# labhamlet/wavjepa

Measured on NVIDIA B200. Metric: WavJEPA-base train 2s-instances/s at 1/2/4/8 B200; tensor-pipe % of peak, higher is better.
Workload: dtype bf16

## Files before the change

include/wavjepa_b200.h:

```cpp
#ifndef WAVJEPA_B200_H
#define WAVJEPA_B200_H

#include <stddef.h>
#include <stdint.h>

#ifdef __cplusplus
extern "C" {
#endif

#define WJ_OK 0
#define WJ_ERR_ARG (-1)
#define WJ_ERR_RUNTIME (-2)
#define WJ_ERR_ARCH (-3)

const char* wj_last_error(void);
int wj_version(void);
long long wj_kernel_launches(void);
int wj_check_device(void);

typedef struct wj_operand {
  const void* ptr;
  int64_t dim[4];
  int64_t stride_bytes[3];
  int32_t seg_width;
// ... 13 lines not shown
  int32_t resid_f32;
  int32_t resid_mod;
  int64_t ld_resid;
  const void* aux;
  int64_t ld_aux;
  int32_t act;
  int32_t _pad;
  const int32_t* out_rows;
  float* colsum;
} wj_epilogue_t;

int wj_gemm_bf16(const wj_operand_t* A, const void* W, int64_t ldw, int L, int batch, int N, int K,
                 const wj_epilogue_t* epi, int block_n, void* stream);

int wj_gemm_dgrad_bf16(const wj_operand_t* A, const void* W, int64_t ldw, int w_rows, int w_cols,
                       const int32_t* seg_col_off, int L, int batch, int N, int K, const wj_epilogue_t* epi,
                       int block_n, void* stream);

int wj_set_deterministic(void* workspace, size_t bytes);

int wj_gemm_option(int key, int value);

int wj_gemm_debug(void* counters);

int wj_gemm_wgrad_bf16(const wj_operand_t* dY, const wj_operand_t* X, int L, int batch, int M, int N, float* out,
                       int64_t ld_out, int accumulate, int splits, void* stream);

int wj_masks_generate(int kind, int batch, int n_times, int in_channels, int channel_based, int n_targets,
                      double ctx_prob, int ctx_len, double tgt_prob, int tgt_len, float cutoff, int min_context_len,
                      uint32_t base_seed, uint32_t row0, uint8_t* ctx_hidden, uint8_t* tgt, uint8_t* vis_hidden,
                      int* attempts, int* err_flag, void* stream);

int wj_mask_indices(const uint8_t* ctx_hidden, const uint8_t* tgt, const uint8_t* vis_hidden, int B, int G, int T,
                    int* n_c, int* n_v, int* n_t, int* cu_c, int* cu_v, int* cu_t, int* totals, int* ctx_rows,
                    int* vis_src, int* vis_pos, int* tgt_vrow, int* tgt_trow, void* stream);

int wj_conv0_moment_count(int Cin);
int wj_conv0_gn_gelu_fwd(const void* x_bf16, const float* w, const float* gamma, const float* beta, int B, int Cin,
                         int L, int C, int k, int stride, float eps, double* moments, float* stats, void* out_bf16,
                         void* dgelu_bf16, void* stream);
int wj_conv0_gn_gelu_bwd(const void* x_bf16, const float* w, const float* gamma, const float* beta, int B, int Cin,
                         int L, int C, int k, int stride, float eps, const double* moments, const float* stats,
                         const void* dy_bf16, const void* dgelu_bf16, void* red_scratch, float* dw, float* dgamma,
                         float* dbeta, void* stream);

int wj_layernorm_fwd(const void* x, int x_is_bf16, const float* gamma, const float* beta, float eps, int M, int D,
// ... 91 lines not shown
```

wavjepa_b200/csrc/attention.cu:

```cuda
#include "common.cuh"

namespace wj {

__device__ __forceinline__ void mma16816(float (&c)[4], const uint32_t (&a)[4], uint32_t b0, uint32_t b1) {
  asm volatile(
      "mma.sync.aligned.m16n8k16.row.col.f32.bf16.bf16.f32 {%0,%1,%2,%3}, {%4,%5,%6,%7}, {%8,%9}, {%0,%1,%2,%3};"
      : "+f"(c[0]), "+f"(c[1]), "+f"(c[2]), "+f"(c[3])
      : "r"(a[0]), "r"(a[1]), "r"(a[2]), "r"(a[3]), "r"(b0), "r"(b1));
}
__device__ __forceinline__ void ldsm_x4_trans(uint32_t& r0, uint32_t& r1, uint32_t& r2, uint32_t& r3, const void* p) {
  asm volatile("ldmatrix.sync.aligned.m8n8.x4.trans.shared.b16 {%0,%1,%2,%3}, [%4];"
               : "=r"(r0), "=r"(r1), "=r"(r2), "=r"(r3)
               : "r"(smem_u32(p)));
}
__device__ __forceinline__ uint32_t lds32(const bf16* p) { return *reinterpret_cast<const uint32_t*>(p); }

__device__ __forceinline__ void ldsm_x4(uint32_t& r0, uint32_t& r1, uint32_t& r2, uint32_t& r3, const void* p) {
  asm volatile("ldmatrix.sync.aligned.m8n8.x4.shared.b16 {%0,%1,%2,%3}, [%4];"
               : "=r"(r0), "=r"(r1), "=r"(r2), "=r"(r3)
               : "r"(smem_u32(p)));
}
__device__ __forceinline__ void cp_async16(void* dst, const void* src) {
  asm volatile("cp.async.cg.shared.global [%0], [%1], 16;" ::"r"(smem_u32(dst)), "l"(src) : "memory");
}
// ... 369 lines not shown

extern "C" int wj_attn_varlen_bwd(const void* qkv_bf16, const void* out_bf16, const void* dout_bf16, const float* lse2,
                                  const int* cu_seqlens, int n_seqs, int max_len, int64_t total_tokens, int D, int H,
                                  void* dqkv_bf16, void* stream) {
  return wj_attn_varlen_bwd_bias(qkv_bf16, out_bf16, dout_bf16, lse2, cu_seqlens, n_seqs, max_len, total_tokens, D, H,
                                 dqkv_bf16, nullptr, stream);
}

static int attn_bwd_bias(const void* qkv_bf16, const void* out_bf16, const void* dout_bf16, const float* lse2,
                         const int* cu_seqlens, int n_seqs, int max_len, int64_t total_tokens, int D, int H,
                         void* dqkv_bf16, float* dbias, void* stream, bool allow_rowstats) {
  if (n_seqs <= 0 || max_len <= 0) return WJ_OK;
  const int dh = D / H;
  if (D % H != 0 || (dh != 32 && dh != 64)) { set_error("wj_attn_varlen_bwd: head dim must be 32 or 64"); return WJ_ERR_ARG; }
  {
    const bool det = wj::det_on();
    const int rc = wj::attn_bwd_tc_launch(qkv_bf16, out_bf16, dout_bf16, lse2, cu_seqlens, n_seqs, max_len, total_tokens, D, H,
                                          dqkv_bf16, det ? nullptr : dbias, WJ_STREAM(stream));
    if (rc < 0) return rc;
    if (rc == 0 && det) {
      if (dbias != nullptr) return wj_colsum(dqkv_bf16, 1, total_tokens, 3 * D, 3 * D, dbias, stream);
      return WJ_OK;
    }
    if (rc == 0) {
      if (dbias != nullptr) return wj_colsum(dout_bf16, 1, total_tokens, D, D, dbias + 2 * D, stream);
      return WJ_OK;
    }
  }
  const int npad = (max_len + 15) & ~15;
  size_t smem = static_cast<size_t>(4) * npad * (dh + 8) * 2 + static_cast<size_t>(2) * ((npad + 63) & ~63) * 4;
  const bool rowstats = allow_rowstats && dh == 64 && smem > 227 * 1024;
  if (rowstats) smem = static_cast<size_t>(4) * npad * (dh + 8) * 2;
  if (smem > 227 * 1024) { set_error("wj_attn_varlen_bwd: sequence of %d tokens (head dim %d) exceeds the shared-memory resident design", max_len, dh); return WJ_ERR_ARG; }
  const float scale = 1.0f / sqrtf(static_cast<float>(dh));
  const float scale_log2 = scale * 1.4426950408889634f;
  dim3 grid(H, n_seqs);
  const bf16* q = reinterpret_cast<const bf16*>(qkv_bf16);
  const bf16* o = reinterpret_cast<const bf16*>(out_bf16);
  const bf16* d_o = reinterpret_cast<const bf16*>(dout_bf16);
  bf16* dq = reinterpret_cast<bf16*>(dqkv_bf16);
  cudaError_t e;
  if (rowstats) {
    e = cudaFuncSetAttribute(attn_bwd_kernel<64, true>, cudaFuncAttributeMaxDynamicSharedMemorySize, static_cast<int>(smem));
    if (e != cudaSuccess) { set_error("attn_bwd attr: %s", cudaGetErrorString(e)); return WJ_ERR_RUNTIME; }
    attn_bwd_kernel<64, true><<<grid, 128, smem, WJ_STREAM(stream)>>>(q, o, d_o, lse2, cu_seqlens, D, H, npad, scale, scale_log2, dq);
  } else if (dh == 64) {
    e = cudaFuncSetAttribute(attn_bwd_kernel<64>, cudaFuncAttributeMaxDynamicSharedMemorySize, static_cast<int>(smem));
    if (e != cudaSuccess) { set_error("attn_bwd attr: %s", cudaGetErrorString(e)); return WJ_ERR_RUNTIME; }
    attn_bwd_kernel<64><<<grid, 128, smem, WJ_STREAM(stream)>>>(q, o, d_o, lse2, cu_seqlens, D, H, npad, scale, scale_log2, dq);
  } else {
// ... 24 lines not shown
```

wavjepa_b200/csrc/attention_tc.cu:

```cuda
#include "common.cuh"

namespace wj {

constexpr int kAtQ = 128;
constexpr int kAtK = 128;

struct AttnTcParams {
  const int* cu;
  int n_seqs, D, H, items;
  float scale_log2;
  bf16* out;
  float* lse2;
  float* out_f32;
};

template <int DH, int KT> struct AttnTcCfg {
  static constexpr int TILE = kAtQ * DH * 2;
  static constexpr int HALVES = KT / 128;
  static constexpr int NW = 4 * HALVES;
  static constexpr int THREADS = (NW + 1) * 32;
  static constexpr int STAGE = 3 * HALVES * TILE;
  static constexpr int STAGES = DH == 32 ? 2 : 1;
  static constexpr int BAR_OFF = STAGES * STAGE;
  static constexpr int ML_OFF = BAR_OFF + 128;
// ... 316 lines not shown
          w.y = pack_bf16x2(__uint_as_float(o[j + 2]) * inv, __uint_as_float(o[j + 3]) * inv);
          w.z = pack_bf16x2(__uint_as_float(o[j + 4]) * inv, __uint_as_float(o[j + 5]) * inv);
          w.w = pack_bf16x2(__uint_as_float(o[j + 6]) * inv, __uint_as_float(o[j + 7]) * inv);
          *reinterpret_cast<uint4*>(op + j) = w;
        }
        if (p.lse2 != nullptr && half == 0) p.lse2[static_cast<long long>(start + row) * p.H + head] = mtot + log2f(lsum);
      }
      }
    }
  }
  tc_fence_before();
  __syncthreads();
  if (warp == NW) {
    tc_fence_after();
    tmem_dealloc(tmem_base, KT);
  }
}

struct AttnBwdParams {
  const int* cu;
  int D, H, items;
  float scale, scale_log2;
  const bf16* out;
  const bf16* dout;
  const float* lse2;
  bf16* dqkv;
  float* dbias;
};

constexpr int kBwdTile = kAtQ * 32 * 2;
constexpr int kBwdPs = 2 * kAtQ * 128;
constexpr int kBwdBarOff = 5 * kBwdTile + 2 * kBwdPs;
constexpr int kBwdCsOff = kBwdBarOff + 128;
constexpr int kBwdCsMaxD = 1024;
constexpr int kBwdSmem = kBwdCsOff + kBwdCsMaxD * 4 + 1024;

__global__ void __launch_bounds__(288, 2) attn_bwd_tc_kernel(const __grid_constant__ CUtensorMap tmQ,
                                                             const __grid_constant__ CUtensorMap tmDO,
                                                             const __grid_constant__ CUtensorMap tmO, const AttnBwdParams p) {
  constexpr int DH = 32;
  constexpr uint32_t SWZ = 4u, SBO = 512u;
  extern __shared__ uint8_t smem_raw[];
  uint8_t* smem = reinterpret_cast<uint8_t*>((reinterpret_cast<uintptr_t>(smem_raw) + 1023) & ~uintptr_t(1023));
  uint8_t* sP = smem + 5 * kBwdTile;
  uint8_t* sDS = sP + kBwdPs;
  uint64_t* bar_load = reinterpret_cast<uint64_t*>(smem + kBwdBarOff);
  uint64_t* bar_s = bar_load + 1;
  uint64_t* bar_p = bar_load + 2;
  uint64_t* bar_g = bar_load + 3;
  uint64_t* bar_done = bar_load + 4;
  uint32_t* tmem_slot = reinterpret_cast<uint32_t*>(bar_load + 5);
  float* s_cs = reinterpret_cast<float*>(smem + kBwdCsOff);
  const int warp = threadIdx.x >> 5, lane = threadIdx.x & 31;
  if (p.dbias != nullptr)
    for (int i = threadIdx.x; i < p.D; i += blockDim.x) s_cs[i] = 0.f;

  if (warp == 8) {
    if (lane == 0) {
      tma_prefetch_desc(&tmQ);
      tma_prefetch_desc(&tmDO);
      tma_prefetch_desc(&tmO);
      mbar_init(bar_load, 1);
      mbar_init(bar_s, 1);
      mbar_init(bar_p, 8);
      mbar_init(bar_g, 1);
      mbar_init(bar_done, 8);
      fence_mbar_init();
    }
    __syncwarp();
    tmem_alloc(tmem_slot, 256);
  }
  tc_fence_before();
  __syncthreads();
  tc_fence_after();
  const uint32_t tmem_base = *tmem_slot;
  const uint32_t tS = tmem_base, tDP = tmem_base + 128, tDV = tmem_base, tDK = tmem_base + 32, tDQ = tmem_base + 64;

  if (warp == 8) {
    if (lane == 0) {
      constexpr uint32_t idesc_g = umma_idesc_bf16(kAtQ, DH, true, true);
      constexpr uint32_t idesc_q = umma_idesc_bf16(kAtQ, DH, false, true);
      const uint32_t sQ = smem_u32(smem), sK = sQ + kBwdTile, sV = sK + kBwdTile, sDO = sV + kBwdTile;
      uint32_t ph_load = 0, ph_p = 0, ph_g = 0, ph_done = 0;
      int it = 0;
      for (int item = blockIdx.x; item < p.items; item += gridDim.x, ++it) {
        const int s = item / p.H, head = item - s * p.H;
        const int start = p.cu[s], n = p.cu[s + 1] - start;
        const int n16 = n > 0 ? (n + 15) & ~15 : 16;
        const uint32_t idesc_s = umma_idesc_bf16(kAtQ, n16, false, false);
        if (it > 0) {
          mbar_wait(bar_g, ph_g);
          ph_g ^= 1;
        }
        mbar_arrive_expect_tx(bar_load, 5 * kBwdTile);
        tma_load_2d(smem, &tmQ, bar_load, head * DH, start);
        tma_load_2d(smem + kBwdTile, &tmQ, bar_load, p.D + head * DH, start);
        tma_load_2d(smem + 2 * kBwdTile, &tmQ, bar_load, 2 * p.D + head * DH, start);
        tma_load_2d(smem + 3 * kBwdTile, &tmDO, bar_load, head * DH, start);
        tma_load_2d(smem + 4 * kBwdTile, &tmO, bar_load, head * DH, start);
        mbar_wait(bar_load, ph_load);
        ph_load ^= 1;
        if (it > 0) {
          mbar_wait(bar_done, ph_done);
          ph_done ^= 1;
        }
        tc_fence_after();
#pragma unroll
        for (int ks = 0; ks < DH / 16; ++ks)
          umma_bf16(tS, umma_smem_desc(sQ + ks * 32, 0, SBO, SWZ), umma_smem_desc(sK + ks * 32, 0, SBO, SWZ), idesc_s, ks > 0 ? 1u : 0u);
#pragma unroll
        for (int ks = 0; ks < DH / 16; ++ks)
          umma_bf16(tDP, umma_smem_desc(sDO + ks * 32, 0, SBO, SWZ), umma_smem_desc(sV + ks * 32, 0, SBO, SWZ), idesc_s, ks > 0 ? 1u : 0u);
        umma_commit(bar_s);
        if (item + gridDim.x < p.items) {
          const int nitem = item + gridDim.x, ns = nitem / p.H, nh = nitem - ns * p.H, nst = p.cu[ns];
          tma_prefetch_2d(&tmQ, nh * DH, nst);
          tma_prefetch_2d(&tmQ, p.D + nh * DH, nst);
          tma_prefetch_2d(&tmQ, 2 * p.D + nh * DH, nst);
          tma_prefetch_2d(&tmDO, nh * DH, nst);
          tma_prefetch_2d(&tmO, nh * DH, nst);
        }
        mbar_wait(bar_p, ph_p);
        ph_p ^= 1;
        tc_fence_after();
        const int steps = n16 / 16;
        const uint64_t dP_mn = umma_smem_desc(smem_u32(sP), kAtQ * 128, 1024, 2u);
        const uint64_t dS_mn = umma_smem_desc(smem_u32(sDS), kAtQ * 128, 1024, 2u);
        const uint64_t bDO = umma_smem_desc(sDO, kBwdTile, SBO, SWZ), bQ = umma_smem_desc(sQ, kBwdTile, SBO, SWZ),
                       bK = umma_smem_desc(sK, kBwdTile, SBO, SWZ);
        for (int kk = 0; kk < steps; ++kk)
          umma_bf16(tDV, dP_mn + static_cast<uint64_t>((kk * 2048) >> 4), bDO + static_cast<uint64_t>((kk * 1024) >> 4), idesc_g, kk > 0 ? 1u : 0u);
        for (int kk = 0; kk < steps; ++kk)
          umma_bf16(tDK, dS_mn + static_cast<uint64_t>((kk * 2048) >> 4), bQ + static_cast<uint64_t>((kk * 1024) >> 4), idesc_g, kk > 0 ? 1u : 0u);
        for (int kk = 0; kk < steps; ++kk) {
          const uint32_t a = smem_u32(sDS) + (kk >> 2) * (kAtQ * 128) + (kk & 3) * 32;
          umma_bf16(tDQ, umma_smem_desc(a, 0, 1024, 2u), bK + static_cast<uint64_t>((kk * 1024) >> 4), idesc_q, kk > 0 ? 1u : 0u);
        }
        umma_commit(bar_g);
      }
    }
  } else {
    const int quad = warp & 3, half = warp >> 2;
    const int row = quad * 32 + lane;
    const uint32_t lane_addr = static_cast<uint32_t>(quad * 32) << 16;
    uint8_t* stage = sP + half * (kAtQ * 128) + quad * 32 * 128;
    uint32_t ph_s = 0, ph_g = 0, ph_l = 0;
    int nstart = 0, nn = 0, n2start = 0, n2n = 0;
    float nlse = 0.f;
    if (blockIdx.x < p.items) {
      const int s = blockIdx.x / p.H;
      nstart = p.cu[s];
      nn = p.cu[s + 1] - nstart;
      if (row < nn) nlse = p.lse2[static_cast<long long>(nstart + row) * p.H + blockIdx.x % p.H];
    }
    if (blockIdx.x + gridDim.x < p.items) {
      const int s = (blockIdx.x + gridDim.x) / p.H;
      n2start = p.cu[s];
      n2n = p.cu[s + 1] - n2start;
    }
    const uint8_t* sOrow = smem + 4 * kBwdTile + row * 64;
    const uint8_t* sDOrow = smem + 3 * kBwdTile + row * 64;
    for (int item = blockIdx.x; item < p.items; item += gridDim.x) {
      const int head = item % p.H;
      const int start = nstart, n = nn;
      const float lse = nlse;
      nstart = n2start;
      nn = n2n;
      if (item + gridDim.x < p.items)
        nlse = row < nn ? p.lse2[static_cast<long long>(nstart + row) * p.H + (item + gridDim.x) % p.H] : 0.f;
      if (item + 2 * gridDim.x < p.items) {
        const int s = (item + 2 * gridDim.x) / p.H;
        n2start = p.cu[s];
        n2n = p.cu[s + 1] - n2start;
      }
      const bool live = row < n;
      mbar_wait(bar_load, ph_l);
      ph_l ^= 1;
      float delta = 0.f;
#pragma unroll
      for (int c = 0; c < 4; ++c) {
        const int o = (c ^ ((row >> 1) & 3)) << 4;
        const uint4 a = *reinterpret_cast<const uint4*>(sOrow + o);
        const uint4 b = *reinterpret_cast<const uint4*>(sDOrow + o);
        const __nv_bfloat162* a2 = reinterpret_cast<const __nv_bfloat162*>(&a);
        const __nv_bfloat162* b2 = reinterpret_cast<const __nv_bfloat162*>(&b);
#pragma unroll
        for (int t = 0; t < 4; ++t) {
          const float2 x = __bfloat1622float2(a2[t]), y = __bfloat1622float2(b2[t]);
          delta += x.x * y.x + x.y * y.y;
        }
      }
      mbar_wait(bar_s, ph_s);
      ph_s ^= 1;
      tc_fence_after();
#pragma unroll 1
      for (int c0 = half * 64; c0 < half * 64 + 64 && c0 < n; c0 += 32) {
        uint32_t sv[32], dv[32];
        tmem_ld_32x32(tS + lane_addr + c0, sv);
        tmem_ld_32x32(tDP + lane_addr + c0, dv);
        tmem_ld_wait();
        const int off = (c0 >> 6) * (kAtQ * 128) + row * 128;
#pragma unroll
        for (int q = 0; q < 4; ++q) {
          uint32_t wp[4], wd[4];
#pragma unroll
          for (int t = 0; t < 4; ++t) {
            const int j = q * 8 + 2 * t;
            const bool k0 = live && c0 + j < n, k1 = live && c0 + j + 1 < n;
            const float p0 = k0 ? ex2_approx(fmaf(__uint_as_float(sv[j]), p.scale_log2, -lse)) : 0.f;
            const float p1 = k1 ? ex2_approx(fmaf(__uint_as_float(sv[j + 1]), p.scale_log2, -lse)) : 0.f;
            wp[t] = pack_bf16x2(p0, p1);
            wd[t] = pack_bf16x2(k0 ? p0 * (__uint_as_float(dv[j]) - delta) : 0.f, k1 ? p1 * (__uint_as_float(dv[j + 1]) - delta) : 0.f);
          }
          const int chunk = ((c0 & 63) >> 3) + q;
          const int o = off + ((chunk ^ (row & 7)) << 4);
          *reinterpret_cast<uint4*>(sP + o) = make_uint4(wp[0], wp[1], wp[2], wp[3]);
          *reinterpret_cast<uint4*>(sDS + o) = make_uint4(wd[0], wd[1], wd[2], wd[3]);
        }
      }
      tc_fence_before();
      fence_proxy_async_smem();
      __syncwarp();
      if (lane == 0) mbar_arrive(bar_p);
      mbar_wait(bar_g, ph_g);
      ph_g ^= 1;
      tc_fence_after();
      const int ntile = half == 0 ? 2 : 1;
#pragma unroll
      for (int t = 0; t < 2; ++t) {
        if (t < ntile) {
          uint32_t g[32];
          tmem_ld_32x32((half == 0 ? (t == 0 ? tDQ : tDV) : tDK) + lane_addr, g);
          tmem_ld_wait();
          const float sc = (half == 0 && t == 1) ? 1.0f : p.scale;
#pragma unroll
          for (int q = 0; q < 4; ++q) {
            uint4 w;
            w.x = pack_bf16x2(__uint_as_float(g[8 * q]) * sc, __uint_as_float(g[8 * q + 1]) * sc);
            w.y = pack_bf16x2(__uint_as_float(g[8 * q + 2]) * sc, __uint_as_float(g[8 * q + 3]) * sc);
            w.z = pack_bf16x2(__uint_as_float(g[8 * q + 4]) * sc, __uint_as_float(g[8 * q + 5]) * sc);
            w.w = pack_bf16x2(__uint_as_float(g[8 * q + 6]) * sc, __uint_as_float(g[8 * q + 7]) * sc);
            *reinterpret_cast<uint4*>(stage + t * 2048 + lane * 64 + ((q ^ ((lane >> 1) & 3)) << 4)) = w;
          }
        }
      }
      if (p.dbias != nullptr && half == 1) {
        uint32_t g[32];
        tmem_ld_32x32(tDQ + lane_addr, g);
        tmem_ld_wait();
        float c32[32];
#pragma unroll
        for (int j = 0; j < 32; j += 2) {
          const uint32_t w = pack_bf16x2(__uint_as_float(g[j]) * p.scale, __uint_as_float(g[j + 1]) * p.scale);
          c32[j] = live ? __uint_as_float(w << 16) : 0.f;
          c32[j + 1] = live ? __uint_as_float(w & 0xffff0000u) : 0.f;
        }
#pragma unroll
        for (int sft = 16; sft >= 1; sft >>= 1) {
          const bool up = (lane & sft) != 0;
#pragma unroll
          for (int i = 0; i < sft; ++i) {
            const float mine = up ? c32[sft + i] : c32[i];
            const float other = up ? c32[i] : c32[sft + i];
            c32[i] = mine + __shfl_xor_sync(0xffffffffu, other, sft);
          }
        }
        atomicAdd(s_cs + head * DH + lane, c32[0]);
      }
      tc_fence_before();
      __syncwarp();
      if (lane == 0) mbar_arrive(bar_done);
      {
        const int rsub = lane >> 2, piece = lane & 3;
#pragma unroll
        for (int t = 0; t < 2; ++t) {
          if (t < ntile) {
            const int col = half == 0 ? (t == 0 ? 0 : 2 * p.D) : p.D;
#pragma unroll
            for (int r0 = 0; r0 < 32; r0 += 8) {
              const int lr = r0 + rsub, r = quad * 32 + lr;
              if (r < n) {
                const uint4 w = *reinterpret_cast<const uint4*>(stage + t * 2048 + lr * 64 + ((piece ^ ((lr >> 1) & 3)) << 4));
                *reinterpret_cast<uint4*>(p.dqkv + static_cast<long long>(start + r) * (3LL * p.D) + col + head * DH + piece * 8) = w;
              }
            }
          }
        }
      }
      __syncwarp();
    }
  }
  tc_fence_before();
  __syncthreads();
  if (p.dbias != nullptr)
    for (int i = threadIdx.x; i < p.D; i += blockDim.x) atomicAdd(p.dbias + i, s_cs[i]);
  if (warp == 8) {
    tc_fence_after();
    tmem_dealloc(tmem_base, 256);
  }
}

typedef CUresult (*PFN_encodeTiledA)(CUtensorMap*, CUtensorMapDataType, cuuint32_t, void*, const cuuint64_t*,
                                     const cuuint64_t*, const cuuint32_t*, const cuuint32_t*, CUtensorMapInterleave,
                                     CUtensorMapSwizzle, CUtensorMapL2promotion, CUtensorMapFloatOOBfill);

int attn_fwd_tc_launch(const void* qkv, const int* cu, int n_seqs, int max_len, long long total_tokens, int D, int H,
                       void* out, float* lse2, cudaStream_t st, float* out_f32) {
  const int dh = D / H;
  if (max_len > 512 || D % 64 != 0 || (dh != 32 && dh != 64) || total_tokens <= 0) return 1;
  static PFN_encodeTiledA enc = nullptr;
  if (enc == nullptr) {
    void* sym = nullptr;
    cudaDriverEntryPointQueryResult qres;
    if (cudaGetDriverEntryPoint("cuTensorMapEncodeTiled", &sym, cudaEnableDefault, &qres) != cudaSuccess ||
        qres != cudaDriverEntryPointSuccess)
      return 1;
    enc = reinterpret_cast<PFN_encodeTiledA>(sym);
  }
// ... 12 lines not shown
  p.out = reinterpret_cast<bf16*>(out); p.lse2 = lse2; p.out_f32 = out_f32;
  auto go = [&](auto kernel, int smem, int ctas, int threads) -> int {
    cudaError_t e = cudaFuncSetAttribute(kernel, cudaFuncAttributeMaxDynamicSharedMemorySize, smem);
    if (e != cudaSuccess) { set_error("attn_fwd_tc attr: %s", cudaGetErrorString(e)); return WJ_ERR_RUNTIME; }
    int grid = ctas * sm_count();
    if (grid > p.items) grid = p.items;
    kernel<<<grid, threads, smem, st>>>(tm, p);
    return check_launch("attn_fwd_tc");
  };
  if (out_f32 != nullptr) {
    if (dh != 64) { set_error("attn_fwd_tc: the fp32-output kernels are built for head dim 64 (got %d)", dh); return WJ_ERR_ARG; }
    if (qt == 4) return go(attn_fwd_tc_kernel<64, 512, true>, AttnTcCfg<64, 512>::SMEM, AttnTcCfg<64, 512>::CTAS, AttnTcCfg<64, 512>::THREADS);
    if (qt == 2) return go(attn_fwd_tc_kernel<64, 256, true>, AttnTcCfg<64, 256>::SMEM, AttnTcCfg<64, 256>::CTAS, AttnTcCfg<64, 256>::THREADS);
    return go(attn_fwd_tc_kernel<64, 128, true>, AttnTcCfg<64, 128>::SMEM, AttnTcCfg<64, 128>::CTAS, AttnTcCfg<64, 128>::THREADS);
  }
  if (dh == 64 && qt == 4) return go(attn_fwd_tc_kernel<64, 512>, AttnTcCfg<64, 512>::SMEM, AttnTcCfg<64, 512>::CTAS, AttnTcCfg<64, 512>::THREADS);
  if (qt == 4) return go(attn_fwd_tc_kernel<32, 512>, AttnTcCfg<32, 512>::SMEM, AttnTcCfg<32, 512>::CTAS, AttnTcCfg<32, 512>::THREADS);
  if (dh == 64 && qt == 1) return go(attn_fwd_tc_kernel<64, 128>, AttnTcCfg<64, 128>::SMEM, AttnTcCfg<64, 128>::CTAS, AttnTcCfg<64, 128>::THREADS);
  if (dh == 64) return go(attn_fwd_tc_kernel<64, 256>, AttnTcCfg<64, 256>::SMEM, AttnTcCfg<64, 256>::CTAS, AttnTcCfg<64, 256>::THREADS);
  if (qt == 1) return go(attn_fwd_tc_kernel<32, 128>, AttnTcCfg<32, 128>::SMEM, AttnTcCfg<32, 128>::CTAS, AttnTcCfg<32, 128>::THREADS);
  return go(attn_fwd_tc_kernel<32, 256>, AttnTcCfg<32, 256>::SMEM, AttnTcCfg<32, 256>::CTAS, AttnTcCfg<32, 256>::THREADS);
}


int attn_bwd_tc_launch(const void* qkv, const void* out, const void* dout, const float* lse2, const int* cu, int n_seqs,
                       int max_len, long long total_tokens, int D, int H, void* dqkv, float* dbias, cudaStream_t st) {
  const int dh = D / H;
  if (max_len > 128 || dh != 32 || D % 8 != 0 || total_tokens <= 0) return 1;
  if (dbias != nullptr && D > kBwdCsMaxD) return 1;
  static PFN_encodeTiledA enc = nullptr;
  if (enc == nullptr) {
    void* sym = nullptr;
    cudaDriverEntryPointQueryResult qres;
    if (cudaGetDriverEntryPoint("cuTensorMapEncodeTiled", &sym, cudaEnableDefault, &qres) != cudaSuccess ||
        qres != cudaDriverEntryPointSuccess)
      return 1;
    enc = reinterpret_cast<PFN_encodeTiledA>(sym);
  }
  CUtensorMap tq, tdo, to;
  cuuint32_t box[2] = {32, kAtQ}, es[2] = {1, 1};
  {
    cuuint64_t dims[2] = {static_cast<cuuint64_t>(3) * D, static_cast<cuuint64_t>(total_tokens)};
    cuuint64_t strides[1] = {static_cast<cuuint64_t>(3) * D * 2};
    if (enc(&tq, CU_TENSOR_MAP_DATA_TYPE_BFLOAT16, 2, const_cast<void*>(qkv), dims, strides, box, es, CU_TENSOR_MAP_INTERLEAVE_NONE,
            CU_TENSOR_MAP_SWIZZLE_64B, CU_TENSOR_MAP_L2_PROMOTION_L2_128B, CU_TENSOR_MAP_FLOAT_OOB_FILL_NONE) != CUDA_SUCCESS)
      return 1;
  }
  {
    cuuint64_t dims[2] = {static_cast<cuuint64_t>(D), static_cast<cuuint64_t>(total_tokens)};
    cuuint64_t strides[1] = {static_cast<cuuint64_t>(D) * 2};
    if (enc(&tdo, CU_TENSOR_MAP_DATA_TYPE_BFLOAT16, 2, const_cast<void*>(dout), dims, strides, box, es, CU_TENSOR_MAP_INTERLEAVE_NONE,
            CU_TENSOR_MAP_SWIZZLE_64B, CU_TENSOR_MAP_L2_PROMOTION_L2_128B, CU_TENSOR_MAP_FLOAT_OOB_FILL_NONE) != CUDA_SUCCESS)
      return 1;
    if (enc(&to, CU_TENSOR_MAP_DATA_TYPE_BFLOAT16, 2, const_cast<void*>(out), dims, strides, box, es, CU_TENSOR_MAP_INTERLEAVE_NONE,
            CU_TENSOR_MAP_SWIZZLE_64B, CU_TENSOR_MAP_L2_PROMOTION_L2_128B, CU_TENSOR_MAP_FLOAT_OOB_FILL_NONE) != CUDA_SUCCESS)
      return 1;
  }
  AttnBwdParams p;
  p.cu = cu; p.D = D; p.H = H; p.items = n_seqs * H;
  p.scale = 1.0f / sqrtf(static_cast<float>(dh));
  p.scale_log2 = p.scale * 1.4426950408889634f;
  p.out = reinterpret_cast<const bf16*>(out); p.dout = reinterpret_cast<const bf16*>(dout); p.lse2 = lse2;
  p.dqkv = reinterpret_cast<bf16*>(dqkv);
  p.dbias = dbias;
  cudaError_t e = cudaFuncSetAttribute(attn_bwd_tc_kernel, cudaFuncAttributeMaxDynamicSharedMemorySize, kBwdSmem);
  if (e != cudaSuccess) { set_error("attn_bwd_tc attr: %s", cudaGetErrorString(e)); return WJ_ERR_RUNTIME; }
  int grid = 2 * sm_count();
  if (grid > p.items) grid = p.items;
  attn_bwd_tc_kernel<<<grid, 288, kBwdSmem, st>>>(tq, tdo, to, p);
  return check_launch("attn_bwd_tc");
}

}
```

Measured before the change: 4992.

## Double-buffer attention backward tiles and keep P in TMEM for dV

Restructures the tcgen05 attention backward kernel so Q/K/V/dO tiles are double-buffered across work items, with a free barrier letting the next item's TMA loads overlap the current item's compute. The output tensor O is no longer TMA-loaded; its row is fetched into registers ahead of use. dV is computed from P held in TMEM (TS-form MMA) instead of staging P in shared memory, and the S/dP operand order is transposed. The dbias column sum over dout is fused into the kernel, replacing a separate colsum launch. Optional clock-based debug counters are added, and the extra TMEM columns, shared memory and barriers add complexity and occupancy risk.

```diff
diff --git a/include/wavjepa_b200.h b/include/wavjepa_b200.h
--- a/include/wavjepa_b200.h
+++ b/include/wavjepa_b200.h
@@ -59,6 +59,8 @@
 int wj_gemm_option(int key, int value);
 
 int wj_gemm_debug(void* counters);
+
+int wj_attn_bwd_debug(void* counters);
 
 int wj_gemm_wgrad_bf16(const wj_operand_t* dY, const wj_operand_t* X, int L, int batch, int M, int N, float* out,
                        int64_t ld_out, int accumulate, int splits, void* stream);
diff --git a/wavjepa_b200/csrc/attention.cu b/wavjepa_b200/csrc/attention.cu
--- a/wavjepa_b200/csrc/attention.cu
+++ b/wavjepa_b200/csrc/attention.cu
@@ -415,10 +415,7 @@
       if (dbias != nullptr) return wj_colsum(dqkv_bf16, 1, total_tokens, 3 * D, 3 * D, dbias, stream);
       return WJ_OK;
     }
-    if (rc == 0) {
-      if (dbias != nullptr) return wj_colsum(dout_bf16, 1, total_tokens, D, D, dbias + 2 * D, stream);
-      return WJ_OK;
-    }
+    if (rc == 0) return WJ_OK;
   }
   const int npad = (max_len + 15) & ~15;
   size_t smem = static_cast<size_t>(4) * npad * (dh + 8) * 2 + static_cast<size_t>(2) * ((npad + 63) & ~63) * 4;
diff --git a/wavjepa_b200/csrc/attention_tc.cu b/wavjepa_b200/csrc/attention_tc.cu
--- a/wavjepa_b200/csrc/attention_tc.cu
+++ b/wavjepa_b200/csrc/attention_tc.cu
@@ -362,49 +362,87 @@
   int D, H, items;
   float scale, scale_log2;
   const bf16* out;
-  const bf16* dout;
   const float* lse2;
   bf16* dqkv;
   float* dbias;
+  long long* dbg;
 };
 
 constexpr int kBwdTile = kAtQ * 32 * 2;
-constexpr int kBwdPs = 2 * kAtQ * 128;
-constexpr int kBwdBarOff = 5 * kBwdTile + 2 * kBwdPs;
-constexpr int kBwdCsOff = kBwdBarOff + 128;
+constexpr int kBwdStage = 4 * kBwdTile;
+constexpr int kBwdDsOff = 2 * kBwdStage;
+constexpr int kBwdDs = 2 * kAtQ * 128;
+constexpr int kBwdBarOff = kBwdDsOff + kBwdDs;
+constexpr int kBwdVecOff = kBwdBarOff + 128;
+constexpr int kBwdCsOff = kBwdVecOff + 2 * kAtQ * 4;
 constexpr int kBwdCsMaxD = 1024;
-constexpr int kBwdSmem = kBwdCsOff + kBwdCsMaxD * 4 + 1024;
+constexpr int kBwdSmem = kBwdCsOff + 2 * kBwdCsMaxD * 4 + 1024;
+static_assert(2 * (kBwdSmem + 1024) <= 228 * 1024, "attn_bwd_tc: two CTAs per SM (1 KB reserved per CTA)");
+static_assert(8 * 4096 <= kBwdStage, "attn_bwd_tc: the epilogue stages each warp's rows in a 4 KB corner of a stage");
+
+__device__ __forceinline__ void tmem_st_32x32_x8(uint32_t taddr, const uint32_t (&w)[8]) {
+  asm volatile("tcgen05.st.sync.aligned.32x32b.x8.b32 [%0], {%1, %2, %3, %4, %5, %6, %7, %8};"
+               ::"r"(taddr), "r"(w[0]), "r"(w[1]), "r"(w[2]), "r"(w[3]), "r"(w[4]), "r"(w[5]), "r"(w[6]), "r"(w[7])
+               : "memory");
+}
+__device__ __forceinline__ void tmem_st_32x32_x4(uint32_t taddr, const uint32_t (&w)[4]) {
+  asm volatile("tcgen05.st.sync.aligned.32x32b.x4.b32 [%0], {%1, %2, %3, %4};"
+               ::"r"(taddr), "r"(w[0]), "r"(w[1]), "r"(w[2]), "r"(w[3])
+               : "memory");
+}
+__device__ __forceinline__ uint32_t clock32() {
+  uint32_t c;
+  asm volatile("mov.u32 %0, %%clock;" : "=r"(c));
+  return c;
+}
+__device__ __forceinline__ void bwd_grad_warps_sync() { asm volatile("bar.sync 1, 256;" ::: "memory"); }
+
+__device__ __forceinline__ float warp_colsum32(float (&c32)[32], int lane) {
+#pragma unroll
+  for (int sft = 16; sft >= 1; sft >>= 1) {
+    const bool up = (lane & sft) != 0;
+#pragma unroll
+    for (int i = 0; i < sft; ++i) {
+      const float mine = up ? c32[sft + i] : c32[i];
+      const float other = up ? c32[i] : c32[sft + i];
+      c32[i] = mine + __shfl_xor_sync(0xffffffffu, other, sft);
+    }
+  }
+  return c32[0];
+}
 
 __global__ void __launch_bounds__(288, 2) attn_bwd_tc_kernel(const __grid_constant__ CUtensorMap tmQ,
-                                                             const __grid_constant__ CUtensorMap tmDO,
-                                                             const __grid_constant__ CUtensorMap tmO, const AttnBwdParams p) {
+                                                             const __grid_constant__ CUtensorMap tmDO, const AttnBwdParams p) {
   constexpr int DH = 32;
   constexpr uint32_t SWZ = 4u, SBO = 512u;
   extern __shared__ uint8_t smem_raw[];
   uint8_t* smem = reinterpret_cast<uint8_t*>((reinterpret_cast<uintptr_t>(smem_raw) + 1023) & ~uintptr_t(1023));
-  uint8_t* sP = smem + 5 * kBwdTile;
-  uint8_t* sDS = sP + kBwdPs;
+  uint8_t* sDS = smem + kBwdDsOff;
   uint64_t* bar_load = reinterpret_cast<uint64_t*>(smem + kBwdBarOff);
-  uint64_t* bar_s = bar_load + 1;
-  uint64_t* bar_p = bar_load + 2;
-  uint64_t* bar_g = bar_load + 3;
-  uint64_t* bar_done = bar_load + 4;
-  uint32_t* tmem_slot = reinterpret_cast<uint32_t*>(bar_load + 5);
+  uint64_t* bar_s = bar_load + 2;
+  uint64_t* bar_p = bar_load + 3;
+  uint64_t* bar_g = bar_load + 4;
+  uint64_t* bar_done = bar_load + 5;
+  uint64_t* bar_free = bar_load + 6;
+  uint32_t* tmem_slot = reinterpret_cast<uint32_t*>(bar_load + 7);
+  float* s_lse = reinterpret_cast<float*>(smem + kBwdVecOff);
+  float* s_delta = s_lse + kAtQ;
   float* s_cs = reinterpret_cast<float*>(smem + kBwdCsOff);
   const int warp = threadIdx.x >> 5, lane = threadIdx.x & 31;
   if (p.dbias != nullptr)
-    for (int i = threadIdx.x; i < p.D; i += blockDim.x) s_cs[i] = 0.f;
+    for (int i = threadIdx.x; i < 2 * p.D; i += blockDim.x) s_cs[i] = 0.f;
 
   if (warp == 8) {
     if (lane == 0) {
       tma_prefetch_desc(&tmQ);
       tma_prefetch_desc(&tmDO);
-      tma_prefetch_desc(&tmO);
       mbar_init(bar_load, 1);
+      mbar_init(bar_load + 1, 1);
       mbar_init(bar_s, 1);
       mbar_init(bar_p, 8);
       mbar_init(bar_g, 1);
       mbar_init(bar_done, 8);
+      mbar_init(bar_free, 8);
       fence_mbar_init();
     }
     __syncwarp();
@@ -414,226 +452,296 @@
   __syncthreads();
   tc_fence_after();
   const uint32_t tmem_base = *tmem_slot;
-  const uint32_t tS = tmem_base, tDP = tmem_base + 128, tDV = tmem_base, tDK = tmem_base + 32, tDQ = tmem_base + 64;
+  const uint32_t tS = tmem_base, tDP = tmem_base + 128, tDV = tmem_base + 128, tDK = tmem_base + 160, tDQ = tmem_base + 192;
 
   if (warp == 8) {
     if (lane == 0) {
-      constexpr uint32_t idesc_g = umma_idesc_bf16(kAtQ, DH, true, true);
-      constexpr uint32_t idesc_q = umma_idesc_bf16(kAtQ, DH, false, true);
-      const uint32_t sQ = smem_u32(smem), sK = sQ + kBwdTile, sV = sK + kBwdTile, sDO = sV + kBwdTile;
-      uint32_t ph_load = 0, ph_p = 0, ph_g = 0, ph_done = 0;
+      constexpr uint32_t idesc_v = umma_idesc_bf16(kAtQ, DH, false, true);
+      constexpr uint32_t idesc_k = umma_idesc_bf16(kAtQ, DH, false, true);
+      constexpr uint32_t idesc_q = umma_idesc_bf16(kAtQ, DH, true, true);
+      auto issue_loads = [&](int item, int stage) {
+        const int s = item / p.H, head = item - s * p.H, start = p.cu[s];
+        uint8_t* b = smem + stage * kBwdStage;
+        mbar_arrive_expect_tx(bar_load + stage, kBwdStage);
+        tma_load_2d(b, &tmQ, bar_load + stage, head * DH, start);
+        tma_load_2d(b + kBwdTile, &tmQ, bar_load + stage, p.D + head * DH, start);
+        tma_load_2d(b + 2 * kBwdTile, &tmQ, bar_load + stage, 2 * p.D + head * DH, start);
+        tma_load_2d(b + 3 * kBwdTile, &tmDO, bar_load + stage, head * DH, start);
+      };
+      uint32_t c_load = 0, c_p = 0, c_done = 0, c_free = 0, tw = 0;
+      const uint32_t c0 = p.dbg ? clock32() : 0;
+      if (blockIdx.x < p.items) issue_loads(blockIdx.x, 0);
+      if (blockIdx.x + gridDim.x < p.items) issue_loads(blockIdx.x + gridDim.x, 1);
+      uint32_t ph_load = 0, ph_p = 0, ph_done = 0, ph_free = 0;
       int it = 0;
       for (int item = blockIdx.x; item < p.items; item += gridDim.x, ++it) {
-        const int s = item / p.H, head = item - s * p.H;
-        const int start = p.cu[s], n = p.cu[s + 1] - start;
+        const int stage = it & 1;
+        const int s = item / p.H;
+        const int n = p.cu[s + 1] - p.cu[s];
         const int n16 = n > 0 ? (n + 15) & ~15 : 16;
         const uint32_t idesc_s = umma_idesc_bf16(kAtQ, n16, false, false);
-        if (it > 0) {
-          mbar_wait(bar_g, ph_g);
-          ph_g ^= 1;
-        }
-        mbar_arrive_expect_tx(bar_load, 5 * kBwdTile);
-        tma_load_2d(smem, &tmQ, bar_load, head * DH, start);
-        tma_load_2d(smem + kBwdTile, &tmQ, bar_load, p.D + head * DH, start);
-        tma_load_2d(smem + 2 * kBwdTile, &tmQ, bar_load, 2 * p.D + head * DH, start);
-        tma_load_2d(smem + 3 * kBwdTile, &tmDO, bar_load, head * DH, start);
-        tma_load_2d(smem + 4 * kBwdTile, &tmO, bar_load, head * DH, start);
-        mbar_wait(bar_load, ph_load);
-        ph_load ^= 1;
+        const uint32_t sQ = smem_u32(smem + stage * kBwdStage), sK = sQ + kBwdTile, sV = sK + kBwdTile, sDO = sV + kBwdTile;
+        if (p.dbg) tw = clock32();
+        mbar_wait(bar_load + stage, (ph_load >> stage) & 1u);
+        ph_load ^= 1u << stage;
+        if (p.dbg) { c_load += clock32() - tw; tw = clock32(); }
         if (it > 0) {
           mbar_wait(bar_done, ph_done);
           ph_done ^= 1;
         }
+        if (p.dbg) c_done += clock32() - tw;
         tc_fence_after();
 #pragma unroll
         for (int ks = 0; ks < DH / 16; ++ks)
-          umma_bf16(tS, umma_smem_desc(sQ + ks * 32, 0, SBO, SWZ), umma_smem_desc(sK + ks * 32, 0, SBO, SWZ), idesc_s, ks > 0 ? 1u : 0u);
+          umma_bf16(tS, umma_smem_desc(sK + ks * 32, 0, SBO, SWZ), umma_smem_desc(sQ + ks * 32, 0, SBO, SWZ), idesc_s, ks > 0 ? 1u : 0u);
 #pragma unroll
         for (int ks = 0; ks < DH / 16; ++ks)
-          umma_bf16(tDP, umma_smem_desc(sDO + ks * 32, 0, SBO, SWZ), umma_smem_desc(sV + ks * 32, 0, SBO, SWZ), idesc_s, ks > 0 ? 1u : 0u);
+          umma_bf16(tDP, umma_smem_desc(sV + ks * 32, 0, SBO, SWZ), umma_smem_desc(sDO + ks * 32, 0, SBO, SWZ), idesc_s, ks > 0 ? 1u : 0u);
         umma_commit(bar_s);
-        if (item + gridDim.x < p.items) {
-          const int nitem = item + gridDim.x, ns = nitem / p.H, nh = nitem - ns * p.H, nst = p.cu[ns];
-          tma_prefetch_2d(&tmQ, nh * DH, nst);
-          tma_prefetch_2d(&tmQ, p.D + nh * DH, nst);
-          tma_prefetch_2d(&tmQ, 2 * p.D + nh * DH, nst);
-          tma_prefetch_2d(&tmDO, nh * DH, nst);
-          tma_prefetch_2d(&tmO, nh * DH, nst);
-        }
+        if (it > 0 && item + gridDim.x < p.items) {
+          if (p.dbg) tw = clock32();
+          mbar_wait(bar_free, ph_free);
+          ph_free ^= 1;
+          if (p.dbg) c_free += clock32() - tw;
+          issue_loads(item + gridDim.x, stage ^ 1);
+        }
+        if (p.dbg) tw = clock32();
         mbar_wait(bar_p, ph_p);
         ph_p ^= 1;
+        if (p.dbg) c_p += clock32() - tw;
         tc_fence_after();
         const int steps = n16 / 16;
-        const uint64_t dP_mn = umma_smem_desc(smem_u32(sP), kAtQ * 128, 1024, 2u);
         const uint64_t dS_mn = umma_smem_desc(smem_u32(sDS), kAtQ * 128, 1024, 2u);
         const uint64_t bDO = umma_smem_desc(sDO, kBwdTile, SBO, SWZ), bQ = umma_smem_desc(sQ, kBwdTile, SBO, SWZ),
                        bK = umma_smem_desc(sK, kBwdTile, SBO, SWZ);
         for (int kk = 0; kk < steps; ++kk)
-          umma_bf16(tDV, dP_mn + static_cast<uint64_t>((kk * 2048) >> 4), bDO + static_cast<uint64_t>((kk * 1024) >> 4), idesc_g, kk > 0 ? 1u : 0u);
-        for (int kk = 0; kk < steps; ++kk)
-          umma_bf16(tDK, dS_mn + static_cast<uint64_t>((kk * 2048) >> 4), bQ + static_cast<uint64_t>((kk * 1024) >> 4), idesc_g, kk > 0 ? 1u : 0u);
+          umma_bf16_ts(tDV, tS + kk * 16, bDO + static_cast<uint64_t>((kk * 1024) >> 4), idesc_v, kk > 0 ? 1u : 0u);
         for (int kk = 0; kk < steps; ++kk) {
           const uint32_t a = smem_u32(sDS) + (kk >> 2) * (kAtQ * 128) + (kk & 3) * 32;
-          umma_bf16(tDQ, umma_smem_desc(a, 0, 1024, 2u), bK + static_cast<uint64_t>((kk * 1024) >> 4), idesc_q, kk > 0 ? 1u : 0u);
-        }
+          umma_bf16(tDK, umma_smem_desc(a, 0, 1024, 2u), bQ + static_cast<uint64_t>((kk * 1024) >> 4), idesc_k, kk > 0 ? 1u : 0u);
+        }
+        for (int kk = 0; kk < steps; ++kk)
+          umma_bf16(tDQ, dS_mn + static_cast<uint64_t>((kk * 2048) >> 4), bK + static_cast<uint64_t>((kk * 1024) >> 4), idesc_q, kk > 0 ? 1u : 0u);
         umma_commit(bar_g);
+      }
+      if (p.dbg) {
+        long long* d = p.dbg + blockIdx.x * 16;
+        d[0] = c_load; d[1] = c_p; d[2] = c_done; d[3] = c_free; d[12] = clock32() - c0; d[14] = it;
       }
     }
   } else {
     const int quad = warp & 3, half = warp >> 2;
     const int row = quad * 32 + lane;
     const uint32_t lane_addr = static_cast<uint32_t>(quad * 32) << 16;
-    uint8_t* stage = sP + half * (kAtQ * 128) + quad * 32 * 128;
-    uint32_t ph_s = 0, ph_g = 0, ph_l = 0;
-    int nstart = 0, nn = 0, n2start = 0, n2n = 0;
+    const bool probe = p.dbg != nullptr && (warp & 3) == 0;
+    uint32_t tw = 0;
+    auto tick = [&](int k) {
+      const uint32_t now = clock32();
+      if (lane == 0) atomicAdd(reinterpret_cast<unsigned long long*>(p.dbg + blockIdx.x * 16 + (half == 0 ? 4 : 8) + k),
+                               static_cast<unsigned long long>(now - tw));
+      tw = now;
+    };
+    int nstart = 0, nn = 0;
+    struct Row64 { uint4 c[4]; };
     float nlse = 0.f;
-    if (blockIdx.x < p.items) {
-      const int s = blockIdx.x / p.H;
+    Row64 no = {};
+    auto bounds = [&](int item) {
+      const int s = item / p.H;
       nstart = p.cu[s];
       nn = p.cu[s + 1] - nstart;
-      if (row < nn) nlse = p.lse2[static_cast<long long>(nstart + row) * p.H + blockIdx.x % p.H];
-    }
-    if (blockIdx.x + gridDim.x < p.items) {
-      const int s = (blockIdx.x + gridDim.x) / p.H;
-      n2start = p.cu[s];
-      n2n = p.cu[s + 1] - n2start;
-    }
-    const uint8_t* sOrow = smem + 4 * kBwdTile + row * 64;
-    const uint8_t* sDOrow = smem + 3 * kBwdTile + row * 64;
-    for (int item = blockIdx.x; item < p.items; item += gridDim.x) {
+    };
+    auto fetch = [&](int item) {
+      const int head = item % p.H, start = nstart, n = nn;
+      if (half == 0) {
+        const uint4* src = reinterpret_cast<const uint4*>(p.out + static_cast<long long>(start + row) * p.D + head * DH);
+        Row64 r;
+#pragma unroll
+        for (int c = 0; c < 4; ++c) r.c[c] = row < n ? src[c] : make_uint4(0, 0, 0, 0);
+        no = r;
+      } else {
+        nlse = row < n ? p.lse2[static_cast<long long>(start + row) * p.H + head] : 0.f;
+      }
+    };
+    if (blockIdx.x < p.items) {
+      bounds(blockIdx.x);
+      fetch(blockIdx.x);
+    }
+    int it = 0;
+    for (int item = blockIdx.x; item < p.items; item += gridDim.x, ++it) {
+      const int stage = it & 1;
       const int head = item % p.H;
       const int start = nstart, n = nn;
+      const int n16 = n > 0 ? (n + 15) & ~15 : 16;
       const float lse = nlse;
-      nstart = n2start;
-      nn = n2n;
-      if (item + gridDim.x < p.items)
-        nlse = row < nn ? p.lse2[static_cast<long long>(nstart + row) * p.H + (item + gridDim.x) % p.H] : 0.f;
-      if (item + 2 * gridDim.x < p.items) {
-        const int s = (item + 2 * gridDim.x) / p.H;
-        n2start = p.cu[s];
-        n2n = p.cu[s + 1] - n2start;
-      }
-      const bool live = row < n;
-      mbar_wait(bar_load, ph_l);
-      ph_l ^= 1;
-      float delta = 0.f;
-#pragma unroll
-      for (int c = 0; c < 4; ++c) {
-        const int o = (c ^ ((row >> 1) & 3)) << 4;
-        const uint4 a = *reinterpret_cast<const uint4*>(sOrow + o);
-        const uint4 b = *reinterpret_cast<const uint4*>(sDOrow + o);
-        const __nv_bfloat162* a2 = reinterpret_cast<const __nv_bfloat162*>(&a);
-        const __nv_bfloat162* b2 = reinterpret_cast<const __nv_bfloat162*>(&b);
-#pragma unroll
-        for (int t = 0; t < 4; ++t) {
-          const float2 x = __bfloat1622float2(a2[t]), y = __bfloat1622float2(b2[t]);
-          delta += x.x * y.x + x.y * y.y;
-        }
-      }
-      mbar_wait(bar_s, ph_s);
-      ph_s ^= 1;
+      const Row64 o4 = no;
+      if (item + gridDim.x < p.items) bounds(item + gridDim.x);
+      uint8_t* sStage = smem + stage * kBwdStage;
+      tw = probe ? clock32() : 0u;
+      const uint32_t ph = static_cast<uint32_t>(it) & 1u, ph_load = (static_cast<uint32_t>(it) >> 1) & 1u;
+      mbar_wait(bar_load + stage, ph_load);
+      if (probe) tick(0);
+      const uint8_t* sDOrow = sStage + 3 * kBwdTile + row * 64;
+      if (half == 0) {
+        float delta = 0.f;
+#pragma unroll
+        for (int c = 0; c < 4; ++c) {
+          const uint4 b = *reinterpret_cast<const uint4*>(sDOrow + ((c ^ ((row >> 1) & 3)) << 4));
+          const __nv_bfloat162* a2 = reinterpret_cast<const __nv_bfloat162*>(&o4.c[c]);
+          const __nv_bfloat162* b2 = reinterpret_cast<const __nv_bfloat162*>(&b);
+#pragma unroll
+          for (int t = 0; t < 4; ++t) {
+            const float2 x = __bfloat1622float2(a2[t]), y = __bfloat1622float2(b2[t]);
+            delta += x.x * y.x + x.y * y.y;
+          }
+        }
+        s_delta[row] = delta;
+      } else {
+        s_lse[row] = lse;
+      }
+      bwd_grad_warps_sync();
+      if (probe) tick(2);
+      mbar_wait(bar_s, ph);
       tc_fence_after();
+      if (probe) tick(0);
+      if (quad * 32 < n16) {
+        const bool kv = row < n;
+        auto convert = [&](const uint32_t (&sv)[8], const uint32_t (&dv)[8], int q0) {
+          uint32_t wp[4], wd[4];
+#pragma unroll
+          for (int t = 0; t < 4; ++t) {
+            const int j = 2 * t, q = q0 + j;
+            const float2 lq = *reinterpret_cast<const float2*>(s_lse + q), dq = *reinterpret_cast<const float2*>(s_delta + q);
+            const bool k0 = kv && q < n, k1 = kv && q + 1 < n;
+            const float p0 = k0 ? ex2_approx(fmaf(__uint_as_float(sv[j]), p.scale_log2, -lq.x)) : 0.f;
+            const float p1 = k1 ? ex2_approx(fmaf(__uint_as_float(sv[j + 1]), p.scale_log2, -lq.y)) : 0.f;
+            wp[t] = pack_bf16x2(p0, p1);
+            wd[t] = pack_bf16x2(k0 ? p0 * (__uint_as_float(dv[j]) - dq.x) : 0.f, k1 ? p1 * (__uint_as_float(dv[j + 1]) - dq.y) : 0.f);
+          }
+          tmem_st_32x32_x4(tS + lane_addr + (q0 & ~15) + ((q0 & 8) >> 1), wp);
+          const int c = (q0 & 63) >> 3;
+          *reinterpret_cast<uint4*>(sDS + (q0 >> 6) * (kAtQ * 128) + row * 128 + ((c ^ (row & 7)) << 4)) = make_uint4(wd[0], wd[1], wd[2], wd[3]);
+        };
+        const int steps = n16 / 16;
+        uint32_t as[8], ad[8], bs[8], bd[8];
+        if (half < steps) {
+          tmem_ld_32x8(tS + lane_addr + half * 16, as);
+          tmem_ld_32x8(tDP + lane_addr + half * 16, ad);
+          tmem_ld_wait();
+        }
 #pragma unroll 1
-      for (int c0 = half * 64; c0 < half * 64 + 64 && c0 < n; c0 += 32) {
-        uint32_t sv[32], dv[32];
-        tmem_ld_32x32(tS + lane_addr + c0, sv);
-        tmem_ld_32x32(tDP + lane_addr + c0, dv);
-        tmem_ld_wait();
-        const int off = (c0 >> 6) * (kAtQ * 128) + row * 128;
-#pragma unroll
-        for (int q = 0; q < 4; ++q) {
-          uint32_t wp[4], wd[4];
-#pragma unroll
-          for (int t = 0; t < 4; ++t) {
-            const int j = q * 8 + 2 * t;
-            const bool k0 = live && c0 + j < n, k1 = live && c0 + j + 1 < n;
-            const float p0 = k0 ? ex2_approx(fmaf(__uint_as_float(sv[j]), p.scale_log2, -lse)) : 0.f;
-            const float p1 = k1 ? ex2_approx(fmaf(__uint_as_float(sv[j + 1]), p.scale_log2, -lse)) : 0.f;
-            wp[t] = pack_bf16x2(p0, p1);
-            wd[t] = pack_bf16x2(k0 ? p0 * (__uint_as_float(dv[j]) - delta) : 0.f, k1 ? p1 * (__uint_as_float(dv[j + 1]) - delta) : 0.f);
-          }
-          const int chunk = ((c0 & 63) >> 3) + q;
-          const int o = off + ((chunk ^ (row & 7)) << 4);
-          *reinterpret_cast<uint4*>(sP + o) = make_uint4(wp[0], wp[1], wp[2], wp[3]);
-          *reinterpret_cast<uint4*>(sDS + o) = make_uint4(wd[0], wd[1], wd[2], wd[3]);
-        }
-      }
+        for (int kk = half; kk < steps; kk += 2) {
+          tmem_ld_32x8(tS + lane_addr + kk * 16 + 8, bs);
+          tmem_ld_32x8(tDP + lane_addr + kk * 16 + 8, bd);
+          convert(as, ad, kk * 16);
+          tmem_ld_wait();
+          if (kk + 2 < steps) {
+            tmem_ld_32x8(tS + lane_addr + (kk + 2) * 16, as);
+            tmem_ld_32x8(tDP + lane_addr + (kk + 2) * 16, ad);
+          }
+          convert(bs, bd, kk * 16 + 8);
+          tmem_ld_wait();
+        }
+      }
+      tmem_st_wait();
       tc_fence_before();
       fence_proxy_async_smem();
       __syncwarp();
       if (lane == 0) mbar_arrive(bar_p);
-      mbar_wait(bar_g, ph_g);
-      ph_g ^= 1;
+      if (probe) tick(2);
+      if (half == 1) {
+          if (p.dbias != nullptr && quad * 32 < n) {
+            float c32[32];
+  #pragma unroll
+            for (int c = 0; c < 4; ++c) {
+              const uint4 b = *reinterpret_cast<const uint4*>(sDOrow + ((c ^ ((row >> 1) & 3)) << 4));
+              const __nv_bfloat162* b2 = reinterpret_cast<const __nv_bfloat162*>(&b);
+  #pragma unroll
+              for (int t = 0; t < 4; ++t) {
+                const float2 y = __bfloat1622float2(b2[t]);
+                c32[8 * c + 2 * t] = row < n ? y.x : 0.f;
+                c32[8 * c + 2 * t + 1] = row < n ? y.y : 0.f;
+              }
+            }
+            const float cs = warp_colsum32(c32, lane);
+            atomicAdd(s_cs + p.D + head * DH + lane, cs);
+          }
+      }
+      mbar_wait(bar_g, ph);
       tc_fence_after();
+      if (probe) tick(1);
+      const bool any = quad * 32 < n;
+      uint8_t* corner = sStage + warp * 4096;
       const int ntile = half == 0 ? 2 : 1;
-#pragma unroll
-      for (int t = 0; t < 2; ++t) {
-        if (t < ntile) {
-          uint32_t g[32];
-          tmem_ld_32x32((half == 0 ? (t == 0 ? tDQ : tDV) : tDK) + lane_addr, g);
-          tmem_ld_wait();
-          const float sc = (half == 0 && t == 1) ? 1.0f : p.scale;
-#pragma unroll
-          for (int q = 0; q < 4; ++q) {
-            uint4 w;
-            w.x = pack_bf16x2(__uint_as_float(g[8 * q]) * sc, __uint_as_float(g[8 * q + 1]) * sc);
-            w.y = pack_bf16x2(__uint_as_float(g[8 * q + 2]) * sc, __uint_as_float(g[8 * q + 3]) * sc);
-            w.z = pack_bf16x2(__uint_as_float(g[8 * q + 4]) * sc, __uint_as_float(g[8 * q + 5]) * sc);
-            w.w = pack_bf16x2(__uint_as_float(g[8 * q + 6]) * sc, __uint_as_float(g[8 * q + 7]) * sc);
-            *reinterpret_cast<uint4*>(stage + t * 2048 + lane * 64 + ((q ^ ((lane >> 1) & 3)) << 4)) = w;
-          }
-        }
-      }
-      if (p.dbias != nullptr && half == 1) {
-        uint32_t g[32];
-        tmem_ld_32x32(tDQ + lane_addr, g);
-        tmem_ld_wait();
-        float c32[32];
-#pragma unroll
-        for (int j = 0; j < 32; j += 2) {
-          const uint32_t w = pack_bf16x2(__uint_as_float(g[j]) * p.scale, __uint_as_float(g[j + 1]) * p.scale);
-          c32[j] = live ? __uint_as_float(w << 16) : 0.f;
-          c32[j + 1] = live ? __uint_as_float(w & 0xffff0000u) : 0.f;
-        }
-#pragma unroll
-        for (int sft = 16; sft >= 1; sft >>= 1) {
-          const bool up = (lane & sft) != 0;
-#pragma unroll
-          for (int i = 0; i < sft; ++i) {
-            const float mine = up ? c32[sft + i] : c32[i];
-            const float other = up ? c32[i] : c32[sft + i];
-            c32[i] = mine + __shfl_xor_sync(0xffffffffu, other, sft);
-          }
-        }
-        atomicAdd(s_cs + head * DH + lane, c32[0]);
-      }
-      tc_fence_before();
-      __syncwarp();
-      if (lane == 0) mbar_arrive(bar_done);
-      {
-        const int rsub = lane >> 2, piece = lane & 3;
+      if (any) {
 #pragma unroll
         for (int t = 0; t < 2; ++t) {
           if (t < ntile) {
-            const int col = half == 0 ? (t == 0 ? 0 : 2 * p.D) : p.D;
+            uint32_t g[32];
+            tmem_ld_32x32((half == 0 ? (t == 0 ? tDV : tDK) : tDQ) + lane_addr, g);
+            tmem_ld_wait();
+            const float sc = (half == 0 && t == 0) ? 1.0f : p.scale;
+            uint32_t w[16];
+#pragma unroll
+            for (int j = 0; j < 16; ++j) w[j] = pack_bf16x2(__uint_as_float(g[2 * j]) * sc, __uint_as_float(g[2 * j + 1]) * sc);
+#pragma unroll
+            for (int q = 0; q < 4; ++q)
+              *reinterpret_cast<uint4*>(corner + t * 2048 + lane * 64 + ((q ^ ((lane >> 1) & 3)) << 4)) =
+                  make_uint4(w[4 * q], w[4 * q + 1], w[4 * q + 2], w[4 * q + 3]);
+          }
+        }
+        tc_fence_before();
+        __syncwarp();
+        if (lane == 0) mbar_arrive(bar_done);
+        if (half == 1 && p.dbias != nullptr) {
+          float c32[32];
+#pragma unroll
+          for (int q = 0; q < 4; ++q) {
+            const uint4 w = *reinterpret_cast<const uint4*>(corner + lane * 64 + ((q ^ ((lane >> 1) & 3)) << 4));
+            const uint32_t wq[4] = {w.x, w.y, w.z, w.w};
+#pragma unroll
+            for (int j = 0; j < 4; ++j) {
+              c32[8 * q + 2 * j] = row < n ? __uint_as_float(wq[j] << 16) : 0.f;
+              c32[8 * q + 2 * j + 1] = row < n ? __uint_as_float(wq[j] & 0xffff0000u) : 0.f;
+            }
+          }
+          const float cs = warp_colsum32(c32, lane);
+          atomicAdd(s_cs + head * DH + lane, cs);
+        }
+        if (item + gridDim.x < p.items) fetch(item + gridDim.x);
+        const int rsub = lane >> 2, piece = lane & 3;
+#pragma unroll
+        for (int t = 0; t < 2; ++t) {
+          if (t < ntile) {
+            const int col = half == 0 ? (t == 0 ? 2 * p.D : p.D) : 0;
 #pragma unroll
             for (int r0 = 0; r0 < 32; r0 += 8) {
               const int lr = r0 + rsub, r = quad * 32 + lr;
               if (r < n) {
-                const uint4 w = *reinterpret_cast<const uint4*>(stage + t * 2048 + lr * 64 + ((piece ^ ((lr >> 1) & 3)) << 4));
+                const uint4 w = *reinterpret_cast<const uint4*>(corner + t * 2048 + lr * 64 + ((piece ^ ((lr >> 1) & 3)) << 4));
                 *reinterpret_cast<uint4*>(p.dqkv + static_cast<long long>(start + r) * (3LL * p.D) + col + head * DH + piece * 8) = w;
               }
             }
           }
         }
-      }
+      } else {
+        tc_fence_before();
+        __syncwarp();
+        if (lane == 0) mbar_arrive(bar_done);
+        if (item + gridDim.x < p.items) fetch(item + gridDim.x);
+      }
+      fence_proxy_async_smem();
       __syncwarp();
+      if (lane == 0) mbar_arrive(bar_free);
+      if (probe) tick(3);
     }
   }
   tc_fence_before();
   __syncthreads();
   if (p.dbias != nullptr)
-    for (int i = threadIdx.x; i < p.D; i += blockDim.x) atomicAdd(p.dbias + i, s_cs[i]);
+    for (int i = threadIdx.x; i < p.D; i += blockDim.x) {
+      atomicAdd(p.dbias + i, s_cs[i]);
+      atomicAdd(p.dbias + 2 * p.D + i, s_cs[p.D + i]);
+    }
   if (warp == 8) {
     tc_fence_after();
     tmem_dealloc(tmem_base, 256);
@@ -692,6 +800,7 @@
   return go(attn_fwd_tc_kernel<32, 256>, AttnTcCfg<32, 256>::SMEM, AttnTcCfg<32, 256>::CTAS, AttnTcCfg<32, 256>::THREADS);
 }
 
+static long long* g_attn_bwd_dbg = nullptr;
 
 int attn_bwd_tc_launch(const void* qkv, const void* out, const void* dout, const float* lse2, const int* cu, int n_seqs,
                        int max_len, long long total_tokens, int D, int H, void* dqkv, float* dbias, cudaStream_t st) {
@@ -707,7 +816,7 @@
       return 1;
     enc = reinterpret_cast<PFN_encodeTiledA>(sym);
   }
-  CUtensorMap tq, tdo, to;
+  CUtensorMap tq, tdo;
   cuuint32_t box[2] = {32, kAtQ}, es[2] = {1, 1};
   {
     cuuint64_t dims[2] = {static_cast<cuuint64_t>(3) * D, static_cast<cuuint64_t>(total_tokens)};
@@ -722,23 +831,26 @@
     if (enc(&tdo, CU_TENSOR_MAP_DATA_TYPE_BFLOAT16, 2, const_cast<void*>(dout), dims, strides, box, es, CU_TENSOR_MAP_INTERLEAVE_NONE,
             CU_TENSOR_MAP_SWIZZLE_64B, CU_TENSOR_MAP_L2_PROMOTION_L2_128B, CU_TENSOR_MAP_FLOAT_OOB_FILL_NONE) != CUDA_SUCCESS)
       return 1;
-    if (enc(&to, CU_TENSOR_MAP_DATA_TYPE_BFLOAT16, 2, const_cast<void*>(out), dims, strides, box, es, CU_TENSOR_MAP_INTERLEAVE_NONE,
-            CU_TENSOR_MAP_SWIZZLE_64B, CU_TENSOR_MAP_L2_PROMOTION_L2_128B, CU_TENSOR_MAP_FLOAT_OOB_FILL_NONE) != CUDA_SUCCESS)
-      return 1;
   }
   AttnBwdParams p;
   p.cu = cu; p.D = D; p.H = H; p.items = n_seqs * H;
   p.scale = 1.0f / sqrtf(static_cast<float>(dh));
   p.scale_log2 = p.scale * 1.4426950408889634f;
-  p.out = reinterpret_cast<const bf16*>(out); p.dout = reinterpret_cast<const bf16*>(dout); p.lse2 = lse2;
+  p.out = reinterpret_cast<const bf16*>(out); p.lse2 = lse2;
   p.dqkv = reinterpret_cast<bf16*>(dqkv);
   p.dbias = dbias;
+  p.dbg = g_attn_bwd_dbg;
   cudaError_t e = cudaFuncSetAttribute(attn_bwd_tc_kernel, cudaFuncAttributeMaxDynamicSharedMemorySize, kBwdSmem);
   if (e != cudaSuccess) { set_error("attn_bwd_tc attr: %s", cudaGetErrorString(e)); return WJ_ERR_RUNTIME; }
   int grid = 2 * sm_count();
   if (grid > p.items) grid = p.items;
-  attn_bwd_tc_kernel<<<grid, 288, kBwdSmem, st>>>(tq, tdo, to, p);
+  attn_bwd_tc_kernel<<<grid, 288, kBwdSmem, st>>>(tq, tdo, p);
   return check_launch("attn_bwd_tc");
 }
 
 }
+
+extern "C" int wj_attn_bwd_debug(void* counters) {
+  wj::g_attn_bwd_dbg = reinterpret_cast<long long*>(counters);
+  return WJ_OK;
+}
```

Measured after the change: 5047, median of 6. +1.1%, better.
